# Vigilans/GomokuAI

Hardware: AMD Instinct MI355X
Metric: board-evals/s (higher is better)
Workload: dtype int32; 1 GPU; batched AC-automaton position eval (K1), 65536 random-opening boards per GPU, 15x15, inputs resident in HBM; boards_per_gpu=65536, parallelism=boards sharded by rank, no collective, launch=hipGraph replay of the K steps

## Files before the change

gomokuai_amd/csrc/eval_kernel.hip:

```cpp
#include <algorithm>
#include <cstdlib>
#include <vector>

#include "capi_common.h"
#include "host_staging.h"

namespace {

constexpr int kBoardsPerBlock = 16;
constexpr int kGroupBoards = 16;
constexpr int kThreads = 64 * kBoardsPerBlock;
constexpr int kCells = 225;
constexpr int kQueueCap = 448;
constexpr int kMaxBlocksPerCu = 1;
constexpr int kBurstEvery = 12;
static_assert(kBurstEvery >= 1 && kBurstEvery <= kGroupBoards, "every burst of a run needs a board of the run to go with");
[[maybe_unused]] constexpr int kTimelineSlots = 8;

constexpr int kScoreWords = 4 * kCells;
constexpr int kCntWords = 3 * kCells + 1;
constexpr int kZeroWords = kScoreWords + kCntWords;
constexpr int kLineWords = 96;
constexpr int kColBase = 20, kDiagBase = 36, kAntiBase = 65;
#ifndef GMK_K1_TOTALS_COPIES
#define GMK_K1_TOTALS_COPIES 8
#endif
constexpr int kTotalsCopies = GMK_K1_TOTALS_COPIES;
constexpr int kMiscWords = 48;
constexpr int kBoardWords = kZeroWords + kLineWords + kQueueCap + kMiscWords;
static_assert(kZeroWords % 4 == 0 && kBoardWords % 4 == 0, "16-byte alignment of the per-board blocks");
constexpr int kPrefixTableWords = gmk::kPrefixWords;
constexpr int kStaticTableWords = 128 + kLineWords + 512 + 1560 + 2 * kPrefixTableWords + 4;

constexpr int kLaneRecordVecs = 2;
constexpr int kSegPads = 2;
constexpr int kScanSteps = 17;
constexpr int kScanPrefixSyms = 4;

__device__ __forceinline__ int dir_stride(int dir) { return (0x0E100F01u >> (8 * dir)) & 0xFFu; }

__device__ __forceinline__ uint64_t line_symbols(uint32_t line_word, int len) {
    return static_cast<uint64_t>(line_word) | (0xAull << (2 * len));
}

__device__ __forceinline__ const __attribute__((address_space(3))) uint32_t* lds_word(uint32_t byte_address) {
    return reinterpret_cast<const __attribute__((address_space(3))) uint32_t*>(static_cast<uintptr_t>(byte_address));
}

__device__ __forceinline__ const __attribute__((address_space(3))) uint16_t* lds_half(uint32_t byte_address) {
    return reinterpret_cast<const __attribute__((address_space(3))) uint16_t*>(static_cast<uintptr_t>(byte_address));
}

__device__ __forceinline__ __attribute__((address_space(3))) uint32_t* lds_word_rw(uint32_t byte_address) {
    return reinterpret_cast<__attribute__((address_space(3))) uint32_t*>(static_cast<uintptr_t>(byte_address));
}

__device__ __forceinline__ uint32_t dfa_address(uint32_t table_word, uint32_t four) {
    uint32_t addr;
    asm("v_bfi_b32 %0, %1, %2, %3" : "=v"(addr) : "s"(0x3FF3u), "v"(table_word), "v"(four));
    return addr;
}

typedef unsigned short v2u16 __attribute__((ext_vector_type(2)));
__device__ __forceinline__ uint32_t pk_dec_u16(uint32_t word) {
    const v2u16 ones = {1, 1};
    return __builtin_bit_cast(uint32_t, static_cast<v2u16>(__builtin_bit_cast(v2u16, word) - ones));
}

__device__ __forceinline__ void store_saddr(uint32_t byte_offset, int32_t value, unsigned long long base) {
    asm volatile("global_store_dword %0, %1, %2" : : "v"(byte_offset), "v"(value), "s"(base) : "memory");
}

template <int kImm, bool kNt>
__device__ __forceinline__ void store_saddr_imm(uint32_t byte_offset, int32_t value, unsigned long long base) {
    static_assert(kImm >= 0 && kImm < 4096, "the immediate offset of a global store has 13 bits, signed");
    if (kNt) asm volatile("global_store_dword %0, %1, %2 offset:%3 nt" : : "v"(byte_offset), "v"(value), "s"(base), "n"(kImm) : "memory");
    else asm volatile("global_store_dword %0, %1, %2 offset:%3" : : "v"(byte_offset), "v"(value), "s"(base), "n"(kImm) : "memory");
}

__device__ __forceinline__ void wave_phase_fence() {
    __builtin_amdgcn_fence(__ATOMIC_RELEASE, "wavefront");
    __builtin_amdgcn_wave_barrier();
    __builtin_amdgcn_fence(__ATOMIC_ACQUIRE, "wavefront");
// ... 171 lines not shown
                           const uint4* __restrict__ g_stage, int stage_vecs, int trans_words, int record_words,
                           int phase_mask_arg, unsigned long long* __restrict__ prof, unsigned long long* __restrict__ timeline) {
#ifdef GMK_PROFILE
    unsigned long long* const tl_row = timeline ? timeline + (static_cast<size_t>(blockIdx.x) * kBoardsPerBlock + (threadIdx.x >> 6)) * kTimelineSlots : nullptr;
#define GMK_TL(slot, value) do { if (tl_row && (threadIdx.x & 63) == 0) tl_row[slot] = (value); } while (0)
    GMK_TL(0, __builtin_amdgcn_s_memtime());
    unsigned long long tl_last_board = 0, tl_burst_clocks = 0;
    int tl_bursts = 0;
    const int phase_mask = phase_mask_arg;
    unsigned long long t_acc[12] = {0, 0, 0, 0, 0, 0, 0, 0, 0, 0, 0, 0}, t_prev = __builtin_amdgcn_s_memtime();
#define GMK_STAMP(k) do { if (prof) { const unsigned long long t_now_ = __builtin_amdgcn_s_memtime(); t_acc[k] += t_now_ - t_prev; t_prev = t_now_; } } while (0)
#else
    constexpr int phase_mask = 0x7F;
    (void)phase_mask_arg; (void)prof; (void)timeline;
#define GMK_TL(slot, value) do { } while (0)
#ifdef GMK_K1_MARKERS
#define GMK_STAMP(k) asm volatile("; gmk_mark " #k)
#else
#define GMK_STAMP(k) do { } while (0)
#endif
#endif
    extern __shared__ __attribute__((aligned(16))) uint32_t lds[];
    const uint4* s_rec = reinterpret_cast<const uint4*>(lds + trans_words);
    uint32_t* s_jobs = lds + trans_words + record_words;

    const int tid = threadIdx.x;
    const uint4 stage_a = g_stage[min(tid, stage_vecs - 1)], stage_b = g_stage[min(tid + kThreads, stage_vecs - 1)];
    const uint4* lane_record = g_stage + stage_vecs + kLaneRecordVecs * (tid & 63);
    const uint4 lane_lines = lane_record[0], lane_consts = lane_record[1];
    uint32_t* s_pads = s_jobs + 128;
    uint2* s_lut = reinterpret_cast<uint2*>(s_jobs + 128 + kLineWords);
    uint32_t* s_wtab_words = s_jobs + 128 + kLineWords + 512;
    const v4i* s_wtab = reinterpret_cast<const v4i*>(s_wtab_words);
    const uint32_t scan_prefix_at = static_cast<uint32_t>(trans_words + record_words + 128 + kLineWords + 512 + kWtabWords) * 4u;
    const uint32_t root_prefix_at = scan_prefix_at + 4u * kPrefixTableWords;
    uint32_t* s_handout = s_wtab_words + kWtabWords + 2 * kPrefixTableWords;

    const int wave = __builtin_amdgcn_readfirstlane(threadIdx.x >> 6), lane0 = threadIdx.x & 63;
    uint32_t* s_scores = lds + trans_words + record_words + kStaticTableWords + wave * kBoardWords;
    uint32_t* s_cnt = s_scores + kScoreWords;
    uint32_t* s_lines = s_scores + kZeroWords;
    uint32_t* s_queue = s_lines + kLineWords;
    uint32_t* s_misc = s_queue + kQueueCap;
#ifndef GMK_K1_TOTALS_HOT
    uint32_t* const my_totals = s_queue + kQueueCap - 8 * kTotalsCopies + (lane0 & (kTotalsCopies - 1)) * 8;
#else
    uint32_t* const my_totals = s_misc + 4;
#endif

    GMK_STAMP(0);

    const bool planes_out = out_density != nullptr && (phase_mask & 64) && !(phase_mask & 1024);
    int lane = lane0;
    const uint32_t job_a = lane_lines.x, job_b = lane_lines.y;
    const uint32_t line_init_lo = lane_lines.z, line_init_hi = lane_lines.w;
    const uint32_t cell_row4 = lane_consts.x, cell_col = lane_consts.y, norm_a = lane_consts.z, norm_b = lane_consts.w;
    uint32_t* s_rows = s_misc + 16;
    const uint16_t* row_ptr = planes + (lane & 15);
    uint32_t next_black = 0, next_white = 0, cur_black = 0, cur_white = 0;
    auto fetch_row = [&](int b) {
        const uint16_t* p = row_ptr + static_cast<size_t>(min(b, n_boards - 1)) * 32;
        next_black = p[0];
        next_white = p[16];
    };
    auto take_row = [&](int lane_m, int b) -> uint32_t { return lane_m < 16 && b < n_boards ? cur_black | (cur_white << 16) : 0u; };

    const int wg_block = static_cast<int>(blockIdx.x);
    const int wg_g0 = groups_each * wg_block + min(wg_block, groups_extra);
    const int wg_groups = groups_each + (wg_block < groups_extra ? 1 : 0);
    const int wg_first = wg_g0 * kGroupBoards, wg_boards = min(wg_groups * kGroupBoards, n_boards - wg_first);
    auto hand_out = [&]() -> int {
        uint32_t v = 0;
        if (lane0 == 0) v = atomicAdd(s_handout, 1u);
        return __builtin_amdgcn_readfirstlane(static_cast<int>(v));
    };
    int idx = wave, boards_done = 0;
    if (idx < wg_boards) fetch_row(wg_first + idx);
// ... 82 lines not shown
                    const uint32_t at_x = code << (2 * x), at_y = code << y2;
                    row_sym |= at_x;
                    char* const col = reinterpret_cast<char*>(s_lines + x);
                    atomicXor(reinterpret_cast<uint32_t*>(col) + kColBase, at_y);
                    atomicXor(reinterpret_cast<uint32_t*>(col - y4) + (kDiagBase + 14), at_x);
                    atomicXor(reinterpret_cast<uint32_t*>(col + y4) + kAntiBase, at_y);
                }
                if (row_sym) atomicXor(&s_lines[y], row_sym);
            }
            wave_phase_fence();
            GMK_STAMP(1);
        }
#ifdef GMK_PROFILE
        if (boards_done == 0) GMK_TL(2, __builtin_amdgcn_s_memtime());
#endif
        if (boards_done == 0) __syncthreads();
#ifdef GMK_PROFILE
        if (boards_done == 0) GMK_TL(3, __builtin_amdgcn_s_memtime());
        if (live) { tl_bursts = 0; tl_burst_clocks = 0; }
#endif
        if (live) {
            int n_queued = 0;
            if (phase_mask & 2) {
                const int len_a = static_cast<int>(job_a & 31u) - kSegPads, len_b = static_cast<int>(job_b & 31u) - kSegPads;
                uint64_t syms = line_symbols(s_lines[(job_a >> 20) & 127u] >> norm_a, len_a);
                syms |= line_symbols(s_lines[(job_b >> 20) & 127u] >> norm_b, len_b) << (2 * (len_a + kSegPads));
                syms |= 0xAAAAAAAAAAAAAAAAull << (2 * (len_a + len_b + 2 * kSegPads));
                const uint32_t cur = static_cast<uint32_t>(syms) << 2;
                const uint32_t rest = static_cast<uint32_t>(syms >> 28);
                const uint32_t q_base = static_cast<uint32_t>(s_queue - lds) * 4u;
                const uint32_t q_full = q_base + 4u * (kQueueCap - 64);
                uint32_t q_at = q_base;
                uint32_t pend_at = 0, pend_entry = 0;
                bool pend = false;
                auto flush = [&]() { if (pend) *lds_word_rw(pend_at) = pend_entry; };
                auto push = [&](uint32_t word, int step) {
                    const bool emits = word > 0x1FFFFu;
                    const unsigned long long emitters = __ballot(emits);
                    const uint32_t ahead = __builtin_amdgcn_mbcnt_hi(static_cast<uint32_t>(emitters >> 32), __builtin_amdgcn_mbcnt_lo(static_cast<uint32_t>(emitters), 0u));
                    pend = emits;
                    pend_at = q_at + 4u * ahead;
                    pend_entry = (word & ~0x1FFFFu) | (static_cast<uint32_t>(lane) | static_cast<uint32_t>(step) << 6);
                    asm volatile("" : "+v"(pend_at), "+v"(pend_entry));
                    q_at = min(q_at + 4u * static_cast<uint32_t>(__popcll(emitters)), q_full);
                };
                uint32_t tw = *lds_half(scan_prefix_at + __builtin_amdgcn_ubfe(cur, 1, 9));
                __builtin_amdgcn_sched_barrier(0);
                late_piece(0);
                __builtin_amdgcn_sched_barrier(0);
#pragma unroll
                for (int step = kScanPrefixSyms; step < kScanSteps; ++step) {
                    const int nth = step - kScanPrefixSyms + 1;
                    const uint32_t four = step < 15 ? __builtin_amdgcn_ubfe(cur, 2 * step, 4) : __builtin_amdgcn_ubfe(rest, 2 * (step - 15), 4);
                    const uint32_t addr = dfa_address(tw, four);
                    const uint32_t before = tw;
                    tw = *lds_word(addr);
                    flush();
                    __builtin_amdgcn_sched_barrier(0);
                    if (step > kScanPrefixSyms) push(before, step - 1);
                    if (nth < kLatePieces) { late_piece(nth); __builtin_amdgcn_sched_barrier(0); }
                }
                flush();
                push(tw, kScanSteps - 1);
                flush();
                n_queued = static_cast<int>((q_at - q_base) >> 2);
                if (q_at >= q_full) s_misc[2] = 1;
            }
#ifdef GMK_PROFILE
            else {
#pragma unroll
                for (int piece = 0; piece < kLatePieces; ++piece) late_piece(piece);
            }
#endif
            wave_phase_fence();
            GMK_STAMP(2);

            if (phase_mask & 4) {
                uint32_t qe_next = s_queue[min(lane, kQueueCap - 1)];
                for (int m = lane; m < n_queued; m += 64) {
                    const uint32_t qe = qe_next;
                    qe_next = s_queue[min(m + 64, kQueueCap - 1)];
                    const int src_lane = qe & 63, src_step = (qe >> 6) & 31;
                    const uint4 rec_now = s_rec[qe >> 17];
                    const uint32_t ja_now = s_jobs[src_lane * 2], jb_now = s_jobs[src_lane * 2 + 1];
                    const int seg_a = ja_now & 31u;
                    const bool second = src_step >= seg_a;
                    const uint32_t job = second ? jb_now : ja_now;
                    const int pos = src_step - (second ? seg_a : 0);
                    const int dir = (job >> 5) & 3, stride = (job >> 7) & 31;
                    const int cell_at = static_cast<int>((job >> 12) & 255u) + pos * stride;
                    deposit_match(rec_now.x, rec_now.y, cell_at, dir, -stride, s_scores, s_cnt, s_misc, my_totals);
                    if (rec_now.z) deposit_match(rec_now.z, rec_now.w, cell_at, dir, -stride, s_scores, s_cnt, s_misc, my_totals);
                }
            }
            wave_phase_fence();
#ifndef GMK_K1_TOTALS_HOT
            if (lane < 8) {
                const uint32_t* t = s_queue + kQueueCap - 8 * kTotalsCopies + lane;
                uint32_t sum = 0;
#pragma unroll
                for (int c = 0; c < kTotalsCopies; ++c) sum += t[8 * c];
                s_misc[4 + lane] = sum;
            }
#endif
            GMK_STAMP(3);

            int n_cand = 0;
            if (phase_mask & 8) {
                uint32_t any_cnt[4];
    #pragma unroll
                for (int pass = 0; pass < 4; ++pass) {
                    const int qc = min(64 * pass + lane, kCells - 1);
                    any_cnt[pass] = s_cnt[qc] | s_cnt[kCells + qc] | s_cnt[2 * kCells + qc];
                }
    #pragma unroll
// ... 195 lines not shown
        wave_phase_fence();
        GMK_STAMP(9);
#ifdef GMK_PROFILE
        tl_last_board = __builtin_amdgcn_s_memtime();
#endif
        idx = idx_next; ++boards_done;
    }
#ifdef GMK_PROFILE
    GMK_TL(4, tl_last_board);
    GMK_TL(6, static_cast<unsigned long long>(tl_bursts) | static_cast<unsigned long long>(boards_done) << 16);
    GMK_TL(7, tl_burst_clocks);
    GMK_TL(5, __builtin_amdgcn_s_memtime());
    if (prof && lane0 == 0) {
        for (int k = 0; k < 12; ++k) atomicAdd(&prof[k], t_acc[k]);
        atomicAdd(&prof[15], 1ull);
    }
#endif
#undef GMK_STAMP
#undef GMK_TL
}

struct LineJob { int len, x0, y0, dir; };

int lane_tables(uint32_t* jobs_out, uint32_t* pads_out, uint32_t* records_out) {
    std::vector<LineJob> lines;
    for (int i = 0; i < 15; ++i) lines.push_back({15, 0, i, 0});
    for (int i = 0; i < 15; ++i) lines.push_back({15, i, 0, 1});
    for (int d = -10; d <= 10; ++d) lines.push_back({15 - std::abs(d), d > 0 ? d : 0, d > 0 ? 0 : -d, 2});
    for (int k = 4; k <= 24; ++k) { const int x0 = std::min(k, 14); lines.push_back({std::min(k, 28 - k) + 1, x0, k - x0, 3}); }
    std::stable_sort(lines.begin(), lines.end(), [](const LineJob& a, const LineJob& b) { return a.len > b.len; });
    uint32_t jobs[128];
    for (uint32_t& j : jobs) j = static_cast<uint32_t>(kSegPads) | (15u << 20);
    auto pack = [](const LineJob& l) {
        const int line = l.dir == 0 ? l.y0 : l.dir == 1 ? kColBase + l.x0 : l.dir == 2 ? kDiagBase + l.x0 - l.y0 + 14 : kAntiBase + l.x0 + l.y0;
        const int stride = l.dir == 0 ? 1 : l.dir == 1 ? 15 : l.dir == 2 ? 16 : 14;
        return static_cast<uint32_t>((l.len + kSegPads) | (l.dir << 5) | (stride << 7) | ((l.y0 * 15 + l.x0) << 12) | (line << 20));
    };
    int steps = 0;
    for (int lane = 0; lane < 64; ++lane) {
        jobs[lane * 2] = pack(lines[lane]);
        if (lines[lane].len < kScanPrefixSyms) { gmk::set_error("lane jobs: lane %d starts with a line of %d cells, the scan's prefix read takes %d", lane, lines[lane].len, kScanPrefixSyms); return GMK_ERR_STATE; }
        int total = lines[lane].len + kSegPads;
        const int extra = 64 + (63 - lane);
        if (extra < static_cast<int>(lines.size())) { jobs[lane * 2 + 1] = pack(lines[extra]); total += lines[extra].len + kSegPads; }
        steps = std::max(steps, total);
    }
    uint32_t init[kLineWords] = {};
    for (int i = 0; i < 15; ++i) init[i] = init[kColBase + i] = 0x3FFFFFFFu;
    for (int d = 0; d <= 28; ++d) init[kDiagBase + d] = init[kAntiBase + d] = ((1u << (2 * (15 - std::abs(d - 14)))) - 1u) << (2 * std::max(0, d - 14));
    uint32_t consts[64][4];
    for (int lane = 0; lane < 64; ++lane) {
        uint32_t row4 = 0, col = 0;
        for (int pass = 0; pass < 4; ++pass) {
            const int c = std::min(64 * pass + lane, kCells - 1);
            if (64 * pass + lane >= kCells) { row4 |= static_cast<uint32_t>(4 * 16) << (8 * pass); continue; }
            row4 |= static_cast<uint32_t>(4 * (c / 15)) << (8 * pass);
            col |= static_cast<uint32_t>(c % 15) << (8 * pass);
        }
        consts[lane][0] = row4;
        consts[lane][1] = col;
        for (int k = 0; k < 2; ++k) {
            const uint32_t job = jobs[lane * 2 + k], dir = (job >> 5) & 3u, first = (job >> 12) & 255u;
            consts[lane][2 + k] = dir == 2u ? 2u * (first % 15u) : dir == 3u ? 2u * (first / 15u) : 0u;
        }
    }
    for (int i = 0; i < 128; ++i) jobs_out[i] = jobs[i];
    for (int i = 0; i < kLineWords; ++i) pads_out[i] = ~init[i] & 0xAAAAAAAAu;
    for (int lane = 0; lane < 64; ++lane) {
        uint32_t* r = records_out + 8 * lane;
        r[0] = jobs[lane * 2]; r[1] = jobs[lane * 2 + 1];
        r[2] = init[lane]; r[3] = init[std::min(64 + lane, kLineWords - 1)];
        for (int k = 0; k < 4; ++k) r[4 + k] = consts[lane][k];
    }
    if (steps != kScanSteps) { gmk::set_error("lane jobs: %d scan steps, the kernel is built for %d", steps, kScanSteps); return GMK_ERR_STATE; }
    return GMK_OK;
}

int density_weights(int8_t* t ) {
    for (int kind = 0; kind < 2; ++kind)
        for (int dy = -3; dy <= 3; ++dy)
            for (int xo = 0; xo < 15; ++xo)
                for (int j = 0; j < 15; ++j) {
                    if (std::abs(j - xo) > 3) continue;
                    const int w = block_weight(dy, j - xo);
                    t[((static_cast<size_t>(kind) * kWtabDy + dy + 6) * 15 + xo) * 16 + j] = static_cast<int8_t>(kind == 0 ? (w != 0) : w);
                }
    for (int cell = 0; cell < 224; ++cell)
        for (int kt = dens_kt_lo(cell / 32); kt <= dens_kt_hi(cell / 32); ++kt)
            for (int h = 0; h < 2; ++h) {
                const int dy = 2 * kt + h - cell / 15;
                if (dy < -6 || dy > 6) { gmk::set_error("density weight table: dy %d of cell %d out of range", dy, cell); return GMK_ERR_STATE; }
            }
    for (int cell = 0; cell < 224; ++cell)
        for (int dy = -3; dy <= 3; ++dy) {
            const int y = cell / 15 + dy, m = cell / 32;
            if (y < 0 || y > 14) continue;
            if (y / 2 < dens_kt_lo(m) || y / 2 > dens_kt_hi(m)) { gmk::set_error("density weight table: row %d of cell %d is not covered", y, cell); return GMK_ERR_STATE; }
// ... 20 lines not shown

int scan_prefix_table(const gmk::DeviceTables& t, uint32_t start, uint16_t* out ) {
    const std::vector<uint32_t>& tr = t.dev_trans;
    for (uint32_t key = 0; key < 256; ++key) {
        uint32_t row = start;
        bool cells = true, reports = false;
        for (int i = 0; i < kScanPrefixSyms; ++i) {
            const uint32_t sym = (key >> (2 * i)) & 3u;
            if (row % 16 != 0 || row / 4 + sym >= tr.size()) { gmk::set_error("K1 scan prefix: a walk from state %u leaves the table", start / 16); return GMK_ERR_STATE; }
            const uint32_t tw = tr[row / 4 + sym];
            cells = cells && sym != 2u;
            reports = reports || gmk::dev_trans_record(tw) != 0;
            row = gmk::dev_trans_row(tw);
        }
        if (cells && reports) { gmk::set_error("K1 scan prefix: the cells of key 0x%02x report a match within four symbols of state %u", key, start / 16); return GMK_ERR_STATE; }
        out[key] = static_cast<uint16_t>(row);
    }
    return GMK_OK;
}

int build_stage_image(const gmk::DeviceState& st, uint4** d_out, int* stage_vecs) {
    const size_t trans_words = static_cast<size_t>(st.n_states) * 4, record_words = static_cast<size_t>(st.n_records) * 4;
    std::vector<uint32_t> rest(kStaticTableWords + 64 * 4 * kLaneRecordVecs, 0u);
    uint32_t* jobs = rest.data(), *pads = jobs + 128, *lut = pads + kLineWords, *wtab = lut + 512, *scan_prefix = wtab + kWtabWords, *root_prefix = scan_prefix + kPrefixTableWords,
              *handout = root_prefix + kPrefixTableWords, *records = handout + 4;
    int rc = lane_tables(jobs, pads, records);
    if (rc != GMK_OK) return rc;
    for (uint32_t b = 0; b < 256; ++b) { lut[2 * b] = ((b & 15u) * 0x204081u) & 0x01010101u; lut[2 * b + 1] = ((b >> 4) * 0x204081u) & 0x01010101u; }
    rc = density_weights(reinterpret_cast<int8_t*>(wtab));
    if (rc != GMK_OK) return rc;
    handout[0] = 2u * kBoardsPerBlock;
    const gmk::DeviceTables& tables = gmk::production_automaton().device();
    rc = scan_start_row(tables, &handout[1]);
    if (rc != GMK_OK) return rc;
    uint16_t halves[256];
    rc = scan_prefix_table(tables, handout[1], halves);
    if (rc != GMK_OK) return rc;
    if (tables.dev_prefix4.size() != 256) { gmk::set_error("K1 tables: no four-symbol prefix table of the root"); return GMK_ERR_STATE; }
    for (int i = 0; i < kPrefixTableWords; ++i) {
        scan_prefix[i] = static_cast<uint32_t>(halves[2 * i]) | static_cast<uint32_t>(halves[2 * i + 1]) << 16;
        root_prefix[i] = static_cast<uint32_t>(tables.dev_prefix4[2 * i]) | static_cast<uint32_t>(tables.dev_prefix4[2 * i + 1]) << 16;
    }
    const size_t staged_words = trans_words + record_words + kStaticTableWords;
    if (staged_words % 4 != 0) { gmk::set_error("K1 tables: %zu staged words are not whole 16-byte pieces", staged_words); return GMK_ERR_STATE; }
    uint32_t* d = nullptr;
    GMK_HIP_CHECK(hipMalloc(&d, (trans_words + record_words + rest.size()) * sizeof(uint32_t)));
    GMK_HIP_CHECK(hipMemcpy(d, st.d_trans, trans_words * sizeof(uint32_t), hipMemcpyDeviceToDevice));
    GMK_HIP_CHECK(hipMemcpy(d + trans_words, st.d_records, record_words * sizeof(uint32_t), hipMemcpyDeviceToDevice));
    GMK_HIP_CHECK(hipMemcpy(d + trans_words + record_words, rest.data(), rest.size() * sizeof(uint32_t), hipMemcpyHostToDevice));
// ... 71 lines not shown
        unsigned long long h[16];
        GMK_HIP_CHECK(hipDeviceSynchronize());
        GMK_HIP_CHECK(hipMemcpy(h, d_prof, sizeof h, hipMemcpyDeviceToHost));
        (void)hipFree(d_prof);
        const char* names[12] = {"staging", "phase0", "scan", "deposits", "phase3", "phase3b", "rescans", "wait-planes", "phaseD", "phase5", "-", "loop-head"};
        const double boards = static_cast<double>(n), waves = static_cast<double>(h[15] ? h[15] : 1);
        double total = 0;
        for (int k = 0; k < 12; ++k) total += static_cast<double>(h[k]);
        std::fprintf(stderr, "[GMK_EVAL_PROFILE] s_memtime cycles per board (wavefront time; %.0f wavefronts, %.0f cycles each):", waves, total / waves);
        for (int k = 0; k < 12; ++k) if (k != 10) std::fprintf(stderr, " %s %.0f", names[k], static_cast<double>(h[k]) / boards);
        std::fprintf(stderr, "\n");
    }
    return GMK_OK;
}

extern "C" int gmk_eval_launch_info(int n, int* grid, int* block, int* lds_bytes) {
    gmk::DeviceState& st = gmk::device_state();
    if (!st.ready) { gmk::set_error("gmk_init has not succeeded"); return GMK_ERR_STATE; }
    const Launch l = plan_launch(std::max(n, 1), st);
    if (grid) *grid = l.grid;
    if (block) *block = kThreads;
    if (lds_bytes) *lds_bytes = static_cast<int>(l.lds);
    return GMK_OK;
}

extern "C" int gmk_eval_batch_host(const uint16_t* h_planes, int n, int32_t* h_scores, int32_t* h_density,
                                   uint32_t* h_totals, int32_t* h_status) {
    GMK_NEED_INIT();
    if (n < 0 || (n > 0 && !h_planes)) { gmk::set_error("gmk_eval_batch_host: bad arguments"); return GMK_ERR_ARG; }
    if (n == 0) return GMK_OK;
    const size_t nb = static_cast<size_t>(n);
    gmk::Staging st("gmk_eval_batch_host", 0, false);
    uint16_t* d_planes;
    int32_t *d_scores, *d_density, *d_status;
    uint32_t* d_totals;
    st.in(d_planes, h_planes, nb * 32);
    st.out(d_scores, h_scores, nb * 900, true); st.out(d_density, h_density, nb * 900, true); st.out(d_totals, h_totals, nb * 11, true);
    st.out(d_status, h_status, nb, true);
    int rc = st.take();
    if (rc == GMK_OK) rc = gmk_eval_batch(d_planes, n, d_scores, d_density, d_totals, d_status, nullptr);
    if (rc != GMK_OK) return rc;
    GMK_STAGED(st, hipDeviceSynchronize());
    return st.download();
}
```

gomokuai_amd/lib.py:

```python
import ctypes as C
import os

import numpy as np

_HERE = os.path.dirname(os.path.abspath(__file__))
_SO = os.path.join(_HERE, "libgomoku_hip.so")
if os.environ.get("GMK_HIP_LIB") == "prof":
    _SO = os.path.join(_HERE, "libgomoku_hip_prof.so")
elif os.environ.get("GMK_HIP_LIB", "").endswith(".so"):
    _SO = os.environ["GMK_HIP_LIB"]

N = 225


class GmkError(RuntimeError):
    pass


class TrainGemmDesc(C.Structure):
    _fields_ = [("A", C.c_void_p), ("sam", C.c_int64), ("sak", C.c_int64), ("a_floats", C.c_int64),
                ("B", C.c_void_p), ("sbk", C.c_int64), ("sbn", C.c_int64), ("b_floats", C.c_int64),
                ("M", C.c_int32), ("N", C.c_int32), ("K", C.c_int32),
                ("kslab", C.c_int32), ("nz", C.c_int32), ("z0", C.c_int32),
                ("part", C.c_void_p), ("part_floats", C.c_int64),
# ... 8 lines not shown
class TableInfo(C.Structure):
    _fields_ = [("n_patterns", C.c_int32), ("n_states", C.c_int32), ("dat_size", C.c_int32),
                ("max_emissions", C.c_int32), ("trans_words", C.c_int32), ("emit_words", C.c_int32),
                ("invariants", C.c_int32 * 5)]


_lib = None

OPT_NOISE_SAMPLER, OPT_LOCKSTEP, OPT_AZ_LEAVES = 1, 2, 3
OPT_AZ_VCF_DEPTH, OPT_AZ_VCF_BUDGET = 4, 5
OPT_AZ_PROOF = 6
AZ_PROOF_NONE, AZ_PROOF_WINS, AZ_PROOF_LOSES = 0, 1, 2
OPT_AZ_VCF_DEFEND = 7
PVNET_F32, PVNET_BF16 = 0, 1
PVNET_PRECISIONS = {"f32": PVNET_F32, "bf16": PVNET_BF16}
PVNET_SYMMETRIES = {"none": 0, "all": 1, "random": 2}
AZ_MAX_LEAVES = 8
NOISE_SAMPLERS = {"std": 0, "counter": 1}

EXPORTS = [
    "gmk_init", "gmk_shutdown", "gmk_pool_release", "gmk_pool_poison", "gmk_last_error", "gmk_device_info",
    "gmk_tables_info", "gmk_tables_pattern", "gmk_tables_copy", "gmk_tables_copy_dat", "gmk_tables_scan",
    "gmk_synth_boards", "gmk_moves_to_planes",
    "gmk_eval_batch", "gmk_eval_batch_host", "gmk_eval_launch_info",
    "gmk_mcts_create", "gmk_mcts_destroy", "gmk_mcts_set_roots", "gmk_mcts_set_game_ids", "gmk_mcts_run", "gmk_mcts_root_stats",
    "gmk_mcts_alg_bytes", "gmk_mcts_launch_info", "gmk_visits_to_pi", "gmk_mcts_advance", "gmk_mcts_step", "gmk_mcts_step_host", "gmk_mcts_add_root_noise", "gmk_mcts_set_option", "gmk_mcts_reserve", "gmk_selfplay_run", "gmk_samples_from_records",
    "gmk_records_scan", "gmk_records_packed_bytes", "gmk_records_pack", "gmk_records_unpack", "gmk_samples_from_packed",
    "gmk_evalstate_create", "gmk_evalstate_destroy", "gmk_evalstate_reset", "gmk_evalstate_update", "gmk_evalstate_update_host", "gmk_evalstate_read",
    "gmk_az_create", "gmk_az_destroy", "gmk_az_set_roots", "gmk_az_select", "gmk_az_expand", "gmk_az_select_host", "gmk_az_expand_host", "gmk_az_read_node_host", "gmk_az_read_children_host", "gmk_az_set_leaf_host", "gmk_az_rollout_host", "gmk_az_expand_stages_host", "gmk_az_write_stats_host", "gmk_az_step", "gmk_az_root_choice", "gmk_az_step_device", "gmk_az_advance", "gmk_az_set_slots", "gmk_az_live_games", "gmk_az_set_game_ids", "gmk_az_add_root_noise", "gmk_az_set_option", "gmk_az_add_playouts", "gmk_az_playouts_owed", "gmk_az_root_stats", "gmk_az_vcf_stats", "gmk_az_vcf_verdicts_host", "gmk_az_defend_stats", "gmk_az_defend_verdicts_host", "gmk_az_root_proofs", "gmk_az_proof_stats",
    "gmk_az_advance_sampled", "gmk_az_root_choice_sampled", "gmk_move_sample_host",
    "gmk_az_set_gumbel", "gmk_az_advance_gumbel", "gmk_az_root_choice_gumbel",
    "gmk_gumbel_sequence_host", "gmk_gumbel_setup_host", "gmk_gumbel_pick_host", "gmk_gumbel_move_host", "gmk_gumbel_row_host",
    "gmk_samples_from_records_target", "gmk_samples_from_packed_target", "gmk_replay_sample_target",
    "gmk_mcts_advance_sampled", "gmk_selfplay_run_sampled", "gmk_trad_selfplay_run_sampled", "gmk_trad_root_choice_sampled",
    "gmk_trad_create", "gmk_trad_destroy", "gmk_trad_reset_evaluators", "gmk_trad_set_game_ids", "gmk_trad_set_positions", "gmk_trad_run", "gmk_trad_step", "gmk_trad_root_choice", "gmk_trad_step_device", "gmk_trad_add_root_noise", "gmk_trad_set_option", "gmk_trad_reserve", "gmk_trad_root_stats", "gmk_trad_read_evaluators", "gmk_trad_run_poolrave", "gmk_trad_run_rave", "gmk_trad_root_amaf", "gmk_trad_selfplay_run", "gmk_pvnet_create", "gmk_pvnet_destroy", "gmk_pvnet_forward", "gmk_pvnet_set_dense", "gmk_pvnet_evaluate",
    "gmk_pvnet_set_precision", "gmk_pvnet_get_precision", "gmk_bf16_round_host",
    "gmk_pvnet_evaluate_sym", "gmk_pvnet_sym_pick_host",
    "gmk_pattern_policy", "gmk_pattern_policy_host", "gmk_pattern_play",
    "gmk_vcf_solve", "gmk_vcf_solve_host", "gmk_vcf_defend", "gmk_vcf_defend_host",
    "gmk_vcf_threats", "gmk_vcf_threats_host", "gmk_vct_solve", "gmk_vct_solve_host",
    "gmk_match_referee",
    "gmk_mcts_ensemble_merge", "gmk_trad_ensemble_merge", "gmk_ensemble_merge_host",
    "gmk_replay_create", "gmk_replay_destroy", "gmk_replay_reset", "gmk_replay_append", "gmk_replay_append_packed", "gmk_replay_size",
    "gmk_replay_sample", "gmk_replay_draw_host", "gmk_replay_image_bytes", "gmk_replay_snapshot", "gmk_replay_restore", "gmk_replay_image_check_host",
    "gmk_train_create", "gmk_train_destroy", "gmk_train_forward", "gmk_train_grads", "gmk_train_step", "gmk_train_params", "gmk_train_set_params",
    "gmk_train_get_block", "gmk_train_set_block", "gmk_train_set_step_count", "gmk_train_export", "gmk_train_info",
    "gmk_train_kernel_gemm", "gmk_train_kernel_reduce", "gmk_train_kernel_im2col", "gmk_train_kernel_col2im",
# ... 13 lines not shown
def load():
    global _lib
    if _lib is not None:
        return _lib
    _torch_first()
    if not os.path.exists(_SO):
        raise GmkError("libgomoku_hip.so is missing: run `python -m gomokuai_amd.build` "
                       "(there is no CPU fallback for the compute path)")
    L = C.CDLL(_SO)
    vp = C.c_void_p
    L.gmk_last_error.restype = C.c_char_p
    L.gmk_init.argtypes = [C.c_int]
    L.gmk_device_info.argtypes = [C.POINTER(C.c_int), C.POINTER(C.c_size_t), C.c_char_p, C.c_int]
    L.gmk_tables_info.argtypes = [C.POINTER(TableInfo)]
    L.gmk_tables_pattern.argtypes = [C.c_int, C.c_char_p, C.POINTER(C.c_int), C.POINTER(C.c_int), C.POINTER(C.c_int)]
    L.gmk_tables_copy.argtypes = [vp, vp, vp]
    L.gmk_tables_copy_dat.argtypes = [vp, vp, vp]
    L.gmk_tables_scan.argtypes = [vp, C.c_int, vp, vp, C.c_int]
    L.gmk_synth_boards.argtypes = [C.c_uint64, C.c_uint32, C.c_int, C.c_int, vp, C.c_int, vp, vp]
    L.gmk_moves_to_planes.argtypes = [vp, C.c_int, vp, C.c_int, vp]
    L.gmk_eval_batch.argtypes = [vp, C.c_int, vp, vp, vp, vp, vp]
    L.gmk_eval_batch_host.argtypes = [vp, C.c_int, vp, vp, vp, vp]
    L.gmk_eval_launch_info.argtypes = [C.c_int, C.POINTER(C.c_int), C.POINTER(C.c_int), C.POINTER(C.c_int)]
    L.gmk_mcts_create.argtypes = [C.c_int, C.c_int, C.c_double, C.c_int, C.c_uint64, C.POINTER(vp)]
    L.gmk_mcts_destroy.argtypes = [vp]
    L.gmk_mcts_set_roots.argtypes = [vp, vp, vp, C.c_uint32]
    L.gmk_mcts_set_game_ids.argtypes = [vp, vp]
    L.gmk_trad_set_game_ids.argtypes = [vp, vp]
    L.gmk_az_set_game_ids.argtypes = [vp, vp]
    L.gmk_mcts_run.argtypes = [vp, C.c_int, vp]
    L.gmk_mcts_root_stats.argtypes = [vp, vp, vp, vp, vp, vp]
    L.gmk_mcts_alg_bytes.argtypes = [vp, C.POINTER(C.c_uint64)]
    L.gmk_mcts_launch_info.argtypes = [vp, C.POINTER(C.c_int), C.POINTER(C.c_int), C.POINTER(C.c_int)]
    L.gmk_visits_to_pi.argtypes = [vp, C.c_int, vp]
    L.gmk_mcts_advance.argtypes = [vp, vp, vp, vp, vp, vp, C.c_int, vp]
    L.gmk_mcts_step.argtypes = [vp, vp, vp, vp, vp, vp, vp, C.c_int, vp]
    L.gmk_mcts_step_host.argtypes = [vp, vp, C.c_int]
    L.gmk_selfplay_run.argtypes = [vp, C.c_int, C.c_uint32, C.c_int, C.c_int, C.c_float, C.c_float, vp, C.c_int, vp, vp, vp, vp, vp, C.POINTER(C.c_int32), vp]
    L.gmk_mcts_advance_sampled.argtypes = [vp, vp, vp, vp, vp, vp, C.c_int, C.c_int, C.c_int, vp]
    L.gmk_selfplay_run_sampled.argtypes = [vp, C.c_int, C.c_uint32, C.c_int, C.c_int, C.c_float, C.c_float, C.c_int, C.c_int, vp, C.c_int, vp, vp, vp, vp, vp, C.POINTER(C.c_int32), vp]
    L.gmk_trad_root_choice_sampled.argtypes = [vp, vp, vp, C.c_int, C.c_int, C.c_uint64, C.c_uint32, vp]
    L.gmk_mcts_add_root_noise.argtypes = [vp, C.c_float, C.c_float, vp]
    L.gmk_noise_mix_rows.argtypes = [vp, vp, vp, vp, C.c_int, C.c_float, C.c_float, C.c_uint64, vp]
    L.gmk_mcts_set_option.argtypes = [vp, C.c_int, C.c_int]
    L.gmk_mcts_reserve.argtypes = [vp, C.c_int]
    L.gmk_trad_reserve.argtypes = [vp, C.c_int]
# ... 211 lines not shown
def eval_batch_host(planes):
    init()
    planes = np.ascontiguousarray(planes, dtype=np.uint16)
    n = planes.shape[0]
    scores = np.zeros((n, 4, N), dtype=np.int32)
    density = np.zeros((n, 2, 2, N), dtype=np.int32)
    totals = np.zeros((n, 11), dtype=np.uint32)
    status = np.zeros(n, dtype=np.int32)
    _check(load().gmk_eval_batch_host(planes.ctypes.data, n, scores.ctypes.data, density.ctypes.data,
                                      totals.ctypes.data, status.ctypes.data))
    return scores, density, totals, status


def eval_batch(d_planes, n, d_scores=None, d_density=None, d_totals=None, d_status=None, stream=None):
    _check(load().gmk_eval_batch(d_planes, n, d_scores, d_density, d_totals, d_status, stream))


def eval_launch_info(n):
    g, b, l = C.c_int(), C.c_int(), C.c_int()
    _check(load().gmk_eval_launch_info(n, C.byref(g), C.byref(b), C.byref(l)))
    return {"grid": g.value, "block": b.value, "lds_bytes": l.value}


class BatchedMCTS:

    def __init__(self, n_games, playouts_capacity=800, c_puct=5.0, c_rollouts=5, seed=DEFAULT_SEED, node_capacity=None):
        init()
        self.n = n_games
        self.cap = node_capacity if node_capacity is not None else playouts_capacity * 225 + 1
        h = C.c_void_p()
        _check(load().gmk_mcts_create(n_games, self.cap, c_puct, c_rollouts, seed, C.byref(h)))
        self.h = h

    def close(self):
        if getattr(self, "h", None) and load is not None:
            load().gmk_mcts_destroy(self.h)
            self.h = None

    __del__ = close

    def set_roots(self, planes, last_moves, first_game_id=0):
        planes = np.ascontiguousarray(planes, dtype=np.uint16)
        last = np.ascontiguousarray(last_moves, dtype=np.int16)
        assert planes.shape == (self.n, 2, 16) and last.shape == (self.n,)
        _check(load().gmk_mcts_set_roots(self.h, planes.ctypes.data, last.ctypes.data, first_game_id))

# ... 1031 lines not shown
```

include/gomoku_hip.h:

```cpp
#ifndef GOMOKU_HIP_H_
#define GOMOKU_HIP_H_
#include <stddef.h>
#include <stdint.h>

#ifdef __cplusplus
extern "C" {
#endif

typedef enum {
    GMK_OK = 0,
    GMK_ERR_NO_DEVICE = -1,
    GMK_ERR_HIP = -2,
    GMK_ERR_ARG = -3,
    GMK_ERR_STATE = -4,
    GMK_ERR_CAPACITY = -5
} gmk_status;

enum { GMK_BOARD_CELLS = 225, GMK_PLANE_WORDS = 16, GMK_TOTALS = 11 };

int gmk_init(int device);
int gmk_shutdown(void);
int gmk_pool_release(void);
int gmk_pool_poison(int on);
const char *gmk_last_error(void);
// ... 4 lines not shown
    int32_t n_states;
    int32_t dat_size;
    int32_t max_emissions;
    int32_t trans_words;
    int32_t emit_words;
    int32_t invariants[5];
} gmk_table_info;
int gmk_tables_info(gmk_table_info *info);
int gmk_tables_pattern(int i, char str[8], int *favour, int *type, int *score);
int gmk_tables_copy(uint32_t *trans, uint16_t *emit_lists, uint32_t *pattern_info);
int gmk_tables_copy_dat(int32_t *base, int32_t *check, int32_t *fail);
int gmk_tables_scan(const uint8_t *codes, int n, int32_t *patterns, int32_t *offsets, int cap);

int gmk_synth_boards(uint64_t seed, uint32_t first_board, int n, int kind,
                     uint8_t *h_moves, int stride, int32_t *h_lens, uint16_t *h_planes);
int gmk_moves_to_planes(const uint8_t *h_moves, int stride, const int32_t *h_lens, int n, uint16_t *h_planes);

int gmk_eval_batch(const uint16_t *d_planes, int n,
                   int32_t *d_scores, int32_t *d_density, uint32_t *d_totals, int32_t *d_status,
                   void *stream);
int gmk_eval_batch_host(const uint16_t *h_planes, int n,
                        int32_t *h_scores, int32_t *h_density, uint32_t *h_totals, int32_t *h_status);
int gmk_eval_launch_info(int n, int *grid, int *block, int *lds_bytes);

typedef struct gmk_evalstate gmk_evalstate;
int gmk_evalstate_create(int n_games, gmk_evalstate **out);
int gmk_evalstate_destroy(gmk_evalstate *e);
int gmk_evalstate_reset(gmk_evalstate *e);
int gmk_evalstate_update(gmk_evalstate *e, const int16_t *d_moves, int moves_per_game, void *stream);
int gmk_evalstate_update_host(gmk_evalstate *e, const int16_t *h_moves, int moves_per_game);
int gmk_evalstate_read(gmk_evalstate *e, int32_t *h_scores, int32_t *h_density, uint32_t *h_pattern_dist, uint32_t *h_compound_dist,
                       int32_t *h_meta, uint8_t *h_record);

typedef struct gmk_mcts gmk_mcts;
int gmk_mcts_create(int n_games, int node_capacity, double c_puct, int c_rollouts, uint64_t seed, gmk_mcts **out);
int gmk_mcts_destroy(gmk_mcts *m);
int gmk_mcts_set_roots(gmk_mcts *m, const uint16_t *h_planes, const int16_t *h_last_move, uint32_t first_game_id);
int gmk_mcts_set_game_ids(gmk_mcts *m, const uint32_t *h_ids);
int gmk_mcts_run(gmk_mcts *m, int playouts, void *stream);
int gmk_mcts_advance(gmk_mcts *m, uint8_t *d_moves, uint16_t *d_visits, int32_t *d_lens, int8_t *d_winner,
                     int32_t *d_unfinished, int reuse_subtree, void *stream);
int gmk_selfplay_run(gmk_mcts *m, int n_total, uint32_t first_game_id, int playouts, int reuse_subtree, float noise_alpha, float noise_epsilon,
                     const uint8_t *h_open_moves, int open_stride, const int32_t *h_open_lens,
                     uint8_t *d_moves, uint16_t *d_visits, int32_t *d_lens, int8_t *d_winner, int32_t *h_steps, void *stream);
int gmk_mcts_step(gmk_mcts* m, const int16_t* d_forced_moves, uint8_t* d_moves, uint16_t* d_visits, int32_t* d_lens,
                  int8_t* d_winner, int32_t* d_unfinished, int reuse_subtree, void* stream);
// ... 280 lines not shown
```

Baseline: 635.0 million board-evals/s.

## Carry decoded cell position in queue entries instead of per-lane job lookups

The scan phase now tracks each lane's current cell, direction and back-step in a running 'place' word, advanced per step with an SDWA add and a DPP jump at the seam between paired lines. Each queue entry stores this decoded position directly, so the deposit phase no longer reads the per-lane job table from LDS or decodes segment, stride and position with branches. The 128-word job table is removed from LDS and the lane pairing is rebuilt so that paired lines share a direction, with a host-side check of every step. This adds a few VALU ops per scan step and relies on inline DPP/SDWA assembly with fixed lane banks.

Measured after the change: 648.0 million board-evals/s, median of 6. 2.0% higher.

```diff
diff --git a/gomokuai_amd/csrc/eval_kernel.hip b/gomokuai_amd/csrc/eval_kernel.hip
--- a/gomokuai_amd/csrc/eval_kernel.hip
+++ b/gomokuai_amd/csrc/eval_kernel.hip
@@ -30,12 +30,14 @@
 constexpr int kBoardWords = kZeroWords + kLineWords + kQueueCap + kMiscWords;
 static_assert(kZeroWords % 4 == 0 && kBoardWords % 4 == 0, "16-byte alignment of the per-board blocks");
 constexpr int kPrefixTableWords = gmk::kPrefixWords;
-constexpr int kStaticTableWords = 128 + kLineWords + 512 + 1560 + 2 * kPrefixTableWords + 4;
+constexpr int kStaticTableWords = kLineWords + 512 + 1560 + 2 * kPrefixTableWords + 4;
 
 constexpr int kLaneRecordVecs = 2;
 constexpr int kSegPads = 2;
 constexpr int kScanSteps = 17;
 constexpr int kScanPrefixSyms = 4;
+constexpr int kPairedLanes = 8, kFirstPairedLane = 64 - kPairedLanes;
+constexpr int kSeamStepLong = 8 + kSegPads, kSeamStepShort = 7 + kSegPads;
 
 __device__ __forceinline__ int dir_stride(int dir) { return (0x0E100F01u >> (8 * dir)) & 0xFFu; }
 
@@ -59,6 +61,26 @@
     uint32_t addr;
     asm("v_bfi_b32 %0, %1, %2, %3" : "=v"(addr) : "s"(0x3FF3u), "v"(table_word), "v"(four));
     return addr;
+}
+
+__device__ __forceinline__ uint32_t place_advance(uint32_t place, uint32_t lines_word) {
+    uint32_t next;
+    asm("v_add_u32_sdwa %0, %1, %2 dst_sel:DWORD dst_unused:UNUSED_PAD src0_sel:DWORD src1_sel:BYTE_3" : "=v"(next) : "v"(place), "v"(lines_word));
+    return next;
+}
+
+template <int kFirstLane>
+__device__ __forceinline__ uint32_t place_jump(uint32_t place, int jump) {
+    static_assert(kFirstLane >= 0 && kFirstLane < 64 && kFirstLane % 4 == 0, "four lanes of one DPP bank");
+    constexpr int kRow = kFirstLane / 16, kBank = (kFirstLane % 16) / 4;
+    asm("s_nop 1\n\tv_add_u32_dpp %0, %1, %0 quad_perm:[0,1,2,3] row_mask:%2 bank_mask:%3" : "+v"(place) : "v"(jump), "n"(1 << kRow), "n"(1 << kBank));
+    return place;
+}
+
+__device__ __forceinline__ uint32_t queue_entry(uint32_t table_word, uint32_t place) {
+    uint32_t entry;
+    asm("v_bfi_b32 %0, %1, %2, %3" : "=v"(entry) : "s"(0x1FFFFu), "v"(place), "v"(table_word));
+    return entry;
 }
 
 typedef unsigned short v2u16 __attribute__((ext_vector_type(2)));
@@ -276,17 +298,17 @@
 #endif
     extern __shared__ __attribute__((aligned(16))) uint32_t lds[];
     const uint4* s_rec = reinterpret_cast<const uint4*>(lds + trans_words);
-    uint32_t* s_jobs = lds + trans_words + record_words;
+    uint32_t* s_static = lds + trans_words + record_words;
 
     const int tid = threadIdx.x;
     const uint4 stage_a = g_stage[min(tid, stage_vecs - 1)], stage_b = g_stage[min(tid + kThreads, stage_vecs - 1)];
     const uint4* lane_record = g_stage + stage_vecs + kLaneRecordVecs * (tid & 63);
     const uint4 lane_lines = lane_record[0], lane_consts = lane_record[1];
-    uint32_t* s_pads = s_jobs + 128;
-    uint2* s_lut = reinterpret_cast<uint2*>(s_jobs + 128 + kLineWords);
-    uint32_t* s_wtab_words = s_jobs + 128 + kLineWords + 512;
+    uint32_t* s_pads = s_static;
+    uint2* s_lut = reinterpret_cast<uint2*>(s_static + kLineWords);
+    uint32_t* s_wtab_words = s_static + kLineWords + 512;
     const v4i* s_wtab = reinterpret_cast<const v4i*>(s_wtab_words);
-    const uint32_t scan_prefix_at = static_cast<uint32_t>(trans_words + record_words + 128 + kLineWords + 512 + kWtabWords) * 4u;
+    const uint32_t scan_prefix_at = static_cast<uint32_t>(trans_words + record_words + kLineWords + 512 + kWtabWords) * 4u;
     const uint32_t root_prefix_at = scan_prefix_at + 4u * kPrefixTableWords;
     uint32_t* s_handout = s_wtab_words + kWtabWords + 2 * kPrefixTableWords;
 
@@ -306,7 +328,7 @@
 
     const bool planes_out = out_density != nullptr && (phase_mask & 64) && !(phase_mask & 1024);
     int lane = lane0;
-    const uint32_t job_a = lane_lines.x, job_b = lane_lines.y;
+    const uint32_t lines_word = lane_lines.x, place_word = lane_lines.y;
     const uint32_t line_init_lo = lane_lines.z, line_init_hi = lane_lines.w;
     const uint32_t cell_row4 = lane_consts.x, cell_col = lane_consts.y, norm_a = lane_consts.z, norm_b = lane_consts.w;
     uint32_t* s_rows = s_misc + 16;
@@ -435,25 +457,33 @@
         if (live) {
             int n_queued = 0;
             if (phase_mask & 2) {
-                const int len_a = static_cast<int>(job_a & 31u) - kSegPads, len_b = static_cast<int>(job_b & 31u) - kSegPads;
-                uint64_t syms = line_symbols(s_lines[(job_a >> 20) & 127u] >> norm_a, len_a);
-                syms |= line_symbols(s_lines[(job_b >> 20) & 127u] >> norm_b, len_b) << (2 * (len_a + kSegPads));
+                const int len_a = static_cast<int>(lines_word & 31u) - kSegPads, len_b = static_cast<int>((lines_word >> 5) & 31u) - kSegPads;
+                uint64_t syms = line_symbols(s_lines[(lines_word >> 10) & 127u] >> norm_a, len_a);
+                syms |= line_symbols(s_lines[(lines_word >> 17) & 127u] >> norm_b, len_b) << (2 * (len_a + kSegPads));
                 syms |= 0xAAAAAAAAAAAAAAAAull << (2 * (len_a + len_b + 2 * kSegPads));
                 const uint32_t cur = static_cast<uint32_t>(syms) << 2;
                 const uint32_t rest = static_cast<uint32_t>(syms >> 28);
                 const uint32_t q_base = static_cast<uint32_t>(s_queue - lds) * 4u;
-                const uint32_t q_full = q_base + 4u * (kQueueCap - 64);
+                constexpr int kQueueFlagAt = kQueueCap - 64;
+                const uint32_t q_full = q_base + 4u * kQueueFlagAt;
+                static_assert(kQueueFlagAt > 0 && (kQueueFlagAt - 1) + 64 < kQueueCap, "the deposits' read one round ahead stays inside the queue");
                 uint32_t q_at = q_base;
                 uint32_t pend_at = 0, pend_entry = 0;
                 bool pend = false;
                 auto flush = [&]() { if (pend) *lds_word_rw(pend_at) = pend_entry; };
+                uint32_t place = place_word;
+                const int seam_jump = __builtin_amdgcn_sbfe(static_cast<int>(place_word), 17, 10);
                 auto push = [&](uint32_t word, int step) {
                     const bool emits = word > 0x1FFFFu;
                     const unsigned long long emitters = __ballot(emits);
                     const uint32_t ahead = __builtin_amdgcn_mbcnt_hi(static_cast<uint32_t>(emitters >> 32), __builtin_amdgcn_mbcnt_lo(static_cast<uint32_t>(emitters), 0u));
                     pend = emits;
                     pend_at = q_at + 4u * ahead;
-                    pend_entry = (word & ~0x1FFFFu) | (static_cast<uint32_t>(lane) | static_cast<uint32_t>(step) << 6);
+                    if (step > kScanPrefixSyms) place = place_advance(place, lines_word);
+                    static_assert(kPairedLanes == 8, "two banks of four lanes: the long first lines in front");
+                    if (step == kSeamStepShort) place = place_jump<kFirstPairedLane + 4>(place, seam_jump);
+                    if (step == kSeamStepLong) place = place_jump<kFirstPairedLane>(place, seam_jump);
+                    pend_entry = queue_entry(word, place);
                     asm volatile("" : "+v"(pend_at), "+v"(pend_entry));
                     q_at = min(q_at + 4u * static_cast<uint32_t>(__popcll(emitters)), q_full);
                 };
@@ -489,21 +519,15 @@
             GMK_STAMP(2);
 
             if (phase_mask & 4) {
-                uint32_t qe_next = s_queue[min(lane, kQueueCap - 1)];
+                uint32_t qe_next = s_queue[lane];
                 for (int m = lane; m < n_queued; m += 64) {
                     const uint32_t qe = qe_next;
-                    qe_next = s_queue[min(m + 64, kQueueCap - 1)];
-                    const int src_lane = qe & 63, src_step = (qe >> 6) & 31;
+                    qe_next = s_queue[m + 64];
                     const uint4 rec_now = s_rec[qe >> 17];
-                    const uint32_t ja_now = s_jobs[src_lane * 2], jb_now = s_jobs[src_lane * 2 + 1];
-                    const int seg_a = ja_now & 31u;
-                    const bool second = src_step >= seg_a;
-                    const uint32_t job = second ? jb_now : ja_now;
-                    const int pos = src_step - (second ? seg_a : 0);
-                    const int dir = (job >> 5) & 3, stride = (job >> 7) & 31;
-                    const int cell_at = static_cast<int>((job >> 12) & 255u) + pos * stride;
-                    deposit_match(rec_now.x, rec_now.y, cell_at, dir, -stride, s_scores, s_cnt, s_misc, my_totals);
-                    if (rec_now.z) deposit_match(rec_now.z, rec_now.w, cell_at, dir, -stride, s_scores, s_cnt, s_misc, my_totals);
+                    const int cell_at = qe & 511u, dir = (qe >> 9) & 3u;
+                    const int back_step = __builtin_amdgcn_sbfe(static_cast<int>(qe), 11, 6);
+                    deposit_match(rec_now.x, rec_now.y, cell_at, dir, back_step, s_scores, s_cnt, s_misc, my_totals);
+                    if (rec_now.z) deposit_match(rec_now.z, rec_now.w, cell_at, dir, back_step, s_scores, s_cnt, s_misc, my_totals);
                 }
             }
             wave_phase_fence();
@@ -745,28 +769,48 @@
 
 struct LineJob { int len, x0, y0, dir; };
 
-int lane_tables(uint32_t* jobs_out, uint32_t* pads_out, uint32_t* records_out) {
+int lane_tables(uint32_t* pads_out, uint32_t* records_out) {
     std::vector<LineJob> lines;
     for (int i = 0; i < 15; ++i) lines.push_back({15, 0, i, 0});
     for (int i = 0; i < 15; ++i) lines.push_back({15, i, 0, 1});
     for (int d = -10; d <= 10; ++d) lines.push_back({15 - std::abs(d), d > 0 ? d : 0, d > 0 ? 0 : -d, 2});
     for (int k = 4; k <= 24; ++k) { const int x0 = std::min(k, 14); lines.push_back({std::min(k, 28 - k) + 1, x0, k - x0, 3}); }
     std::stable_sort(lines.begin(), lines.end(), [](const LineJob& a, const LineJob& b) { return a.len > b.len; });
-    uint32_t jobs[128];
-    for (uint32_t& j : jobs) j = static_cast<uint32_t>(kSegPads) | (15u << 20);
-    auto pack = [](const LineJob& l) {
-        const int line = l.dir == 0 ? l.y0 : l.dir == 1 ? kColBase + l.x0 : l.dir == 2 ? kDiagBase + l.x0 - l.y0 + 14 : kAntiBase + l.x0 + l.y0;
-        const int stride = l.dir == 0 ? 1 : l.dir == 1 ? 15 : l.dir == 2 ? 16 : 14;
-        return static_cast<uint32_t>((l.len + kSegPads) | (l.dir << 5) | (stride << 7) | ((l.y0 * 15 + l.x0) << 12) | (line << 20));
-    };
+    if (lines.size() != 64 + kPairedLanes) { gmk::set_error("lane lines: %zu lines for 64 lanes and %d second lines", lines.size(), kPairedLanes); return GMK_ERR_STATE; }
+    auto line_word = [](const LineJob& l) { return l.dir == 0 ? l.y0 : l.dir == 1 ? kColBase + l.x0 : l.dir == 2 ? kDiagBase + l.x0 - l.y0 + 14 : kAntiBase + l.x0 + l.y0; };
+    auto stride_of = [](int dir) { return dir == 0 ? 1 : dir == 1 ? 15 : dir == 2 ? 16 : 14; };
+    auto first_cell = [](const LineJob& l) { return l.y0 * 15 + l.x0; };
+    auto second_line = [](int lane) { return lane < kFirstPairedLane ? -1 : lane < kFirstPairedLane + 4 ? lane + 12 : lane + 4; };
+    uint32_t lines_words[64], place_words[64];
     int steps = 0;
     for (int lane = 0; lane < 64; ++lane) {
-        jobs[lane * 2] = pack(lines[lane]);
-        if (lines[lane].len < kScanPrefixSyms) { gmk::set_error("lane jobs: lane %d starts with a line of %d cells, the scan's prefix read takes %d", lane, lines[lane].len, kScanPrefixSyms); return GMK_ERR_STATE; }
-        int total = lines[lane].len + kSegPads;
-        const int extra = 64 + (63 - lane);
-        if (extra < static_cast<int>(lines.size())) { jobs[lane * 2 + 1] = pack(lines[extra]); total += lines[extra].len + kSegPads; }
-        steps = std::max(steps, total);
+        const LineJob& a = lines[lane];
+        const LineJob* b = second_line(lane) < 0 ? nullptr : &lines[second_line(lane)];
+        if (a.len < kScanPrefixSyms) { gmk::set_error("lane lines: lane %d starts with a line of %d cells, the scan's prefix read takes %d", lane, a.len, kScanPrefixSyms); return GMK_ERR_STATE; }
+        if (b && b->dir != a.dir) { gmk::set_error("lane lines: lane %d walks lines of directions %d and %d", lane, a.dir, b->dir); return GMK_ERR_STATE; }
+        const int seg_a = a.len + kSegPads, seg_b = b ? b->len + kSegPads : kSegPads, stride = stride_of(a.dir);
+        if (b && seg_a != (lane < kFirstPairedLane + 4 ? kSeamStepLong : kSeamStepShort)) { gmk::set_error("lane lines: lane %d steps to its second line at step %d", lane, seg_a); return GMK_ERR_STATE; }
+        const int jump = b ? first_cell(*b) - (first_cell(a) + seg_a * stride) : 0;
+        if (jump < -512 || jump > 511) { gmk::set_error("lane lines: lane %d jumps %d cells", lane, jump); return GMK_ERR_STATE; }
+        lines_words[lane] = static_cast<uint32_t>(seg_a | seg_b << 5 | line_word(a) << 10 | (b ? line_word(*b) : 15) << 17 | stride << 24);
+        place_words[lane] = static_cast<uint32_t>(first_cell(a) + kScanPrefixSyms * stride) | static_cast<uint32_t>(a.dir) << 9 | (static_cast<uint32_t>(-stride) & 63u) << 11
+                            | (static_cast<uint32_t>(jump) & 1023u) << 17;
+        steps = std::max(steps, seg_a + (b ? seg_b : 0));
+        uint32_t place = place_words[lane];
+        const int jump_field = static_cast<int>(place_words[lane] << 5) >> 22;
+        for (int step = kScanPrefixSyms; step < kScanSteps; ++step) {
+            if (step > kScanPrefixSyms) place += lines_words[lane] >> 24;
+            if (step == kSeamStepShort && lane >= kFirstPairedLane + 4) place += static_cast<uint32_t>(jump_field);
+            if (step == kSeamStepLong && lane >= kFirstPairedLane && lane < kFirstPairedLane + 4) place += static_cast<uint32_t>(jump_field);
+            const bool second = b && step >= seg_a;
+            const LineJob& l = second ? *b : a;
+            const int cell = first_cell(l) + (step - (second ? seg_a : 0)) * stride_of(l.dir);
+            const uint32_t want = static_cast<uint32_t>(cell) | static_cast<uint32_t>(l.dir) << 9 | (static_cast<uint32_t>(-stride_of(l.dir)) & 63u) << 11;
+            if (cell < 0 || cell > 511 || (place & 0x1FFFFu) != want) {
+                gmk::set_error("lane lines: lane %d step %d carries place 0x%05x, the plain statement gives 0x%05x", lane, step, place & 0x1FFFFu, want);
+                return GMK_ERR_STATE;
+            }
+        }
     }
     uint32_t init[kLineWords] = {};
     for (int i = 0; i < 15; ++i) init[i] = init[kColBase + i] = 0x3FFFFFFFu;
@@ -783,19 +827,18 @@
         consts[lane][0] = row4;
         consts[lane][1] = col;
         for (int k = 0; k < 2; ++k) {
-            const uint32_t job = jobs[lane * 2 + k], dir = (job >> 5) & 3u, first = (job >> 12) & 255u;
-            consts[lane][2 + k] = dir == 2u ? 2u * (first % 15u) : dir == 3u ? 2u * (first / 15u) : 0u;
-        }
-    }
-    for (int i = 0; i < 128; ++i) jobs_out[i] = jobs[i];
+            const int at = k == 0 ? lane : second_line(lane);
+            consts[lane][2 + k] = at < 0 ? 0u : lines[at].dir == 2 ? 2u * static_cast<uint32_t>(lines[at].x0) : lines[at].dir == 3 ? 2u * static_cast<uint32_t>(lines[at].y0) : 0u;
+        }
+    }
     for (int i = 0; i < kLineWords; ++i) pads_out[i] = ~init[i] & 0xAAAAAAAAu;
     for (int lane = 0; lane < 64; ++lane) {
         uint32_t* r = records_out + 8 * lane;
-        r[0] = jobs[lane * 2]; r[1] = jobs[lane * 2 + 1];
+        r[0] = lines_words[lane]; r[1] = place_words[lane];
         r[2] = init[lane]; r[3] = init[std::min(64 + lane, kLineWords - 1)];
         for (int k = 0; k < 4; ++k) r[4 + k] = consts[lane][k];
     }
-    if (steps != kScanSteps) { gmk::set_error("lane jobs: %d scan steps, the kernel is built for %d", steps, kScanSteps); return GMK_ERR_STATE; }
+    if (steps != kScanSteps) { gmk::set_error("lane lines: %d scan steps, the kernel is built for %d", steps, kScanSteps); return GMK_ERR_STATE; }
     return GMK_OK;
 }
 
@@ -862,9 +905,9 @@
 int build_stage_image(const gmk::DeviceState& st, uint4** d_out, int* stage_vecs) {
     const size_t trans_words = static_cast<size_t>(st.n_states) * 4, record_words = static_cast<size_t>(st.n_records) * 4;
     std::vector<uint32_t> rest(kStaticTableWords + 64 * 4 * kLaneRecordVecs, 0u);
-    uint32_t* jobs = rest.data(), *pads = jobs + 128, *lut = pads + kLineWords, *wtab = lut + 512, *scan_prefix = wtab + kWtabWords, *root_prefix = scan_prefix + kPrefixTableWords,
+    uint32_t* pads = rest.data(), *lut = pads + kLineWords, *wtab = lut + 512, *scan_prefix = wtab + kWtabWords, *root_prefix = scan_prefix + kPrefixTableWords,
               *handout = root_prefix + kPrefixTableWords, *records = handout + 4;
-    int rc = lane_tables(jobs, pads, records);
+    int rc = lane_tables(pads, records);
     if (rc != GMK_OK) return rc;
     for (uint32_t b = 0; b < 256; ++b) { lut[2 * b] = ((b & 15u) * 0x204081u) & 0x01010101u; lut[2 * b + 1] = ((b >> 4) * 0x204081u) & 0x01010101u; }
     rc = density_weights(reinterpret_cast<int8_t*>(wtab));
@@ -982,6 +1025,12 @@
     if (block) *block = kThreads;
     if (lds_bytes) *lds_bytes = static_cast<int>(l.lds);
     return GMK_OK;
+}
+
+extern "C" int gmk_eval_lane_records(uint32_t* records) {
+    if (!records) { gmk::set_error("gmk_eval_lane_records: bad arguments"); return GMK_ERR_ARG; }
+    uint32_t pads[kLineWords];
+    return lane_tables(pads, records);
 }
 
 extern "C" int gmk_eval_batch_host(const uint16_t* h_planes, int n, int32_t* h_scores, int32_t* h_density,
diff --git a/gomokuai_amd/lib.py b/gomokuai_amd/lib.py
--- a/gomokuai_amd/lib.py
+++ b/gomokuai_amd/lib.py
@@ -54,7 +54,7 @@
     "gmk_init", "gmk_shutdown", "gmk_pool_release", "gmk_pool_poison", "gmk_last_error", "gmk_device_info",
     "gmk_tables_info", "gmk_tables_pattern", "gmk_tables_copy", "gmk_tables_copy_dat", "gmk_tables_scan",
     "gmk_synth_boards", "gmk_moves_to_planes",
-    "gmk_eval_batch", "gmk_eval_batch_host", "gmk_eval_launch_info",
+    "gmk_eval_batch", "gmk_eval_batch_host", "gmk_eval_launch_info", "gmk_eval_lane_records",
     "gmk_mcts_create", "gmk_mcts_destroy", "gmk_mcts_set_roots", "gmk_mcts_set_game_ids", "gmk_mcts_run", "gmk_mcts_root_stats",
     "gmk_mcts_alg_bytes", "gmk_mcts_launch_info", "gmk_visits_to_pi", "gmk_mcts_advance", "gmk_mcts_step", "gmk_mcts_step_host", "gmk_mcts_add_root_noise", "gmk_mcts_set_option", "gmk_mcts_reserve", "gmk_selfplay_run", "gmk_samples_from_records",
     "gmk_records_scan", "gmk_records_packed_bytes", "gmk_records_pack", "gmk_records_unpack", "gmk_samples_from_packed",
@@ -114,6 +114,7 @@
     L.gmk_eval_batch.argtypes = [vp, C.c_int, vp, vp, vp, vp, vp]
     L.gmk_eval_batch_host.argtypes = [vp, C.c_int, vp, vp, vp, vp]
     L.gmk_eval_launch_info.argtypes = [C.c_int, C.POINTER(C.c_int), C.POINTER(C.c_int), C.POINTER(C.c_int)]
+    L.gmk_eval_lane_records.argtypes = [vp]
     L.gmk_mcts_create.argtypes = [C.c_int, C.c_int, C.c_double, C.c_int, C.c_uint64, C.POINTER(vp)]
     L.gmk_mcts_destroy.argtypes = [vp]
     L.gmk_mcts_set_roots.argtypes = [vp, vp, vp, C.c_uint32]
@@ -371,6 +372,12 @@
     return {"grid": g.value, "block": b.value, "lds_bytes": l.value}
 
 
+def eval_lane_records():
+    rec = np.zeros((64, 8), dtype=np.uint32)
+    _check(load().gmk_eval_lane_records(rec.ctypes.data))
+    return rec
+
+
 class BatchedMCTS:
 
     def __init__(self, n_games, playouts_capacity=800, c_puct=5.0, c_rollouts=5, seed=DEFAULT_SEED, node_capacity=None):
diff --git a/include/gomoku_hip.h b/include/gomoku_hip.h
--- a/include/gomoku_hip.h
+++ b/include/gomoku_hip.h
@@ -50,6 +50,7 @@
 int gmk_eval_batch_host(const uint16_t *h_planes, int n,
                         int32_t *h_scores, int32_t *h_density, uint32_t *h_totals, int32_t *h_status);
 int gmk_eval_launch_info(int n, int *grid, int *block, int *lds_bytes);
+int gmk_eval_lane_records(uint32_t *records );
 
 typedef struct gmk_evalstate gmk_evalstate;
 int gmk_evalstate_create(int n_games, gmk_evalstate **out);
```
